# DongSky/few-shot-vit

Hardware: AMD Instinct MI355X
Metric: episodes_per_sec_5way_5shot_visformer_s (higher is better)
Workload: dtype bf16; 1 GPU; BASELINE configs[1]: Visformer-S (visformer_micro_80) miniImageNet-shaped 5-way 5-shot episodic eval, 15 query/class, 80x80 fp32 NCHW episodes resident in HBM, procedural weights + calibrated BN; images_per_episode=100, encoder_chunk_images=12800, distinct_episode_batches=16, parallelism=episode-parallel x1, one all-reduce of accuracy stats, ranks_seen=1, per_rank_eps=4602.6

## Files before the change

few-shot-vit_amd/csrc/conv3x3_halo.hip:

```cpp
#include <stdlib.h>

#include <type_traits>
#include <utility>

#include "conv_gemm.h"
#include "fsvit_common.h"

namespace FSVIT_NS {

__device__ __attribute__((aligned(256))) unsigned char g_zero_page_halo[256];
typedef __attribute__((address_space(3))) void* lptrh_t;

__device__ __forceinline__ void hdma1(const void* gsrc, unsigned lds_byte_addr) {
  unsigned keep;
  asm volatile(
      "s_mov_b32 %0, m0\n\t"
      "s_mov_b32 m0, %2\n\t"
      "s_nop 0\n\t"
      "global_load_lds_dwordx4 %1, off\n\t"
      "s_mov_b32 m0, %0"
      : "=&s"(keep)
      : "v"(gsrc), "s"(lds_byte_addr)
      : "memory");
}
__device__ __forceinline__ void hdma2s(unsigned off0, unsigned off1, const void* sbase, unsigned lds0, unsigned lds1) {
  unsigned keep;
  asm volatile(
      "s_mov_b32 %0, m0\n\t"
      "s_mov_b32 m0, %4\n\t"
      "s_nop 0\n\t"
      "global_load_lds_dwordx4 %1, %3\n\t"
      "s_mov_b32 m0, %5\n\t"
      "s_nop 0\n\t"
      "global_load_lds_dwordx4 %2, %3\n\t"
      "s_mov_b32 m0, %0"
      : "=&s"(keep)
      : "v"(off0), "v"(off1), "s"(sbase), "s"(lds0), "s"(lds1)
      : "memory");
}
__device__ __forceinline__ u32x4 hgload16(const void* p) {
  u32x4 v;
  asm volatile("global_load_dwordx4 %0, %1, off" : "=v"(v) : "v"(p) : "memory");
  return v;
}
#define HWAIT(vm) asm volatile("s_waitcnt vmcnt(" #vm ") lgkmcnt(0)" ::: "memory")
__device__ __forceinline__ void hbar() {
  asm volatile("s_barrier" ::: "memory");
  __builtin_amdgcn_sched_barrier(0);
}

template <int CTRL>
__device__ __forceinline__ float quad_xor(float v) {
  return __builtin_bit_cast(float, __builtin_amdgcn_update_dpp(0, __builtin_bit_cast(int, v), CTRL, 0xf, 0xf, true));
}

namespace halo {
constexpr int TR = 8, TW = 40;
constexpr int HR = TR + 2, HP = 44;
constexpr int PLANE = 7168;
constexpr int NPIECE = 7;
constexpr int HBUF = 8 * PLANE;
constexpr int NST = 3, STAGE = 16384;
constexpr int OFF_W = 2 * HBUF;
constexpr int LDS_BYTES = OFF_W + NST * STAGE;
static_assert(LDS_BYTES == 160 * 1024, "the two halo buffers and the weight ring fill the LDS exactly");
}

template <int... I, typename F>
__device__ __forceinline__ void static_for_impl(std::integer_sequence<int, I...>, F&& f) {
  (f(std::integral_constant<int, I>{}), ...);
}
template <int N, typename F>
__device__ __forceinline__ void static_for(F&& f) { static_for_impl(std::make_integer_sequence<int, N>{}, static_cast<F&&>(f)); }

template <int CIN, bool FUSE_TAIL, bool STATS = false>
__global__ __launch_bounds__(512, 2) void conv3x3_halo_kernel(const ConvGemmParams p, const int n_tiles) {
  using namespace halo;
  extern __shared__ __attribute__((aligned(16))) unsigned char smem[];
  constexpr int NH = CIN / 64;
  constexpr int NKM = 9 * NH, NKT = NKM + (FUSE_TAIL ? 1 : 0);
  constexpr int MT = 5, NT = 4;
  const int t = threadIdx.x, lane = t & 63;
  const int wave = __builtin_amdgcn_readfirstlane(t >> 6);
  const int wm = wave >> 1, wn = wave & 1;
  const int lrow = lane & 15, lq = lane >> 4;
  const unsigned lds0 = (unsigned)(size_t)(lptrh_t)smem;
  unsigned char* const wst0 = smem + OFF_W;

  const unsigned char* const Xb = reinterpret_cast<const unsigned char*>(p.x);
  const unsigned char* const Wb = reinterpret_cast<const unsigned char*>(p.w);
  bf16* __restrict__ Y = reinterpret_cast<bf16*>(p.y);
  const int tiles_per_img = p.H / TR;

  const int fr = ((lrow >> 3) & 1) * 2 + ((lrow >> 1) & 1), fc = ((lrow >> 2) & 1) * 2 + (lrow & 1);
  auto blk_r = [&](int i) { return (wm * MT + i) / (TW / 4); };
  auto blk_c = [&](int i) { return (wm * MT + i) % (TW / 4); };
  f32x4 st0[STATS ? NT : 1], st1[STATS ? NT : 1];
#pragma unroll
  for (int j = 0; j < (STATS ? NT : 1); ++j) st0[j] = st1[j] = f32x4{0.f, 0.f, 0.f, 0.f};
  unsigned xb[MT];
#pragma unroll
  for (int i = 0; i < MT; ++i) xb[i] = (unsigned)(((blk_r(i) * 4 + fr) * HP + blk_c(i) * 4 + fc) * 16 + lq * PLANE);
  const int srow = lane >> 3;
  const unsigned schunk = (unsigned)(((lane & 7) ^ srow) << 4);
  unsigned offB[2];
#pragma unroll
  for (int j = 0; j < 2; ++j) {
    const int R = (2 * wave + j) * 8 + srow;
    const int ch = (R & ~31) + 8 * ((R & 15) >> 2) + 4 * ((R >> 4) & 1) + (R & 3);
    offB[j] = (unsigned)ch * (unsigned)(p.Kw * 2) + schunk;
  }
  const unsigned b_rd = (unsigned)((wn * 64 + lrow) * 128);
  const unsigned sw0 = (unsigned)((lq ^ (lrow & 7)) << 4), sw1 = (unsigned)(((4 + lq) ^ (lrow & 7)) << 4);

  auto issue_w = [&](int wk, int stage) {
    const unsigned d = lds0 + OFF_W + stage * STAGE;
    hdma2s(offB[0], offB[1], Wb + (size_t)wk * 128, d + (2 * wave) * 1024, d + (2 * wave + 1) * 1024);
  };
  const int x_rs = p.x_planar ? (CIN / 8) * p.W * 16 : p.W * CIN * 2, x_ps = p.x_planar ? 16 : CIN * 2;
  auto issue_piece = [&](int j, int lane_o, const unsigned char* base, bool top, bool bot, int nb) {
    const int s = j * 64 + lane_o, hr = s / HP, hc = s - hr * HP;
    const bool ok = (base != nullptr) & (s < HR * HP) & (hc >= 1) & (hc <= TW) & !(top & (hr == 0)) & !(bot & (hr == HR - 1));
    const unsigned long a = (unsigned long)base + (unsigned long)(unsigned)(hr * x_rs + (hc - 1) * x_ps);
    const unsigned long z = (unsigned long)g_zero_page_halo;
    hdma1(reinterpret_cast<const void*>(ok ? a : z), lds0 + nb * HBUF + wave * PLANE + j * 1024);
  };
  auto halo_base = [&](int tile, int h) {
    const int bb = tile / tiles_per_img, rr = (tile - bb * tiles_per_img) * TR;
    return Xb + (long)(bb * p.H + rr - 1) * x_rs + (p.x_planar ? (h * 8 + wave) * p.W * 16 : h * 128 + wave * 16);
  };

  f32x4 acc[MT][NT];
#pragma unroll
  for (int i = 0; i < MT; ++i)
#pragma unroll
    for (int j = 0; j < NT; ++j) acc[i][j] = f32x4{0.f, 0.f, 0.f, 0.f};

  int tix = blockIdx.x;
  if (tix >= n_tiles) return;
  const int my_tiles = (n_tiles - tix + (int)gridDim.x - 1) / (int)gridDim.x;
  int steps_left = my_tiles * NKT;

  auto wk_of = [&](int q) { return q >= NKM ? NKM : (NH == 2 ? (q >= 9 ? (q - 9) * 2 + 1 : q * 2) : q); };

  {
    const int r00 = (tix % tiles_per_img) * TR;
    const unsigned char* b0 = halo_base(tix, 0);
#pragma unroll
    for (int j = 0; j < NPIECE; ++j) issue_piece(j, lane, b0, r00 == 0, r00 + TR == p.H, 0);
  }
  issue_w(wk_of(0), 0);
  issue_w(wk_of(1 % NKT), 1);
  HWAIT(0);
  hbar();
  int st_cur = 0, st_pre = 2, q_pre = 2 % NKT;
  int buf = 0;
#define H_STAMP(acc_)

  auto advance = [&]() {
    st_cur = st_cur == NST - 1 ? 0 : st_cur + 1;
    st_pre = st_pre == NST - 1 ? 0 : st_pre + 1;
    q_pre = q_pre == NKT - 1 ? 0 : q_pre + 1;
    --steps_left;
  };

  while (true) {
    const int tnext = tix + (int)gridDim.x;
    const bool has_next = tnext < n_tiles;
    const int b = tix / tiles_per_img, r0 = (tix - b * tiles_per_img) * TR;
    u32x4 xf0[MT], wf0[NT];

#pragma unroll 1
    for (int h = 0; h < NH; ++h) {
      const int n_tix = h + 1 < NH ? tix : (has_next ? tnext : -1), n_h = h + 1 < NH ? h + 1 : 0;
      const unsigned char* nbase = n_tix >= 0 ? halo_base(n_tix, n_h) : nullptr;
      const int n_r0 = n_tix >= 0 ? (n_tix % tiles_per_img) * TR : 0;
      const bool n_top = n_r0 == 0, n_bot = n_r0 + TR == p.H;
      int lane_o = lane;
      asm volatile("" : "+v"(lane_o));
      u32x4 xf1[MT], wf1[NT];
      {
        const unsigned char* wb = wst0 + st_cur * STAGE + b_rd;
#pragma unroll
        for (int j = 0; j < NT; ++j) wf0[j] = *reinterpret_cast<const u32x4*>(wb + j * 2048 + sw0);
#pragma unroll
        for (int i = 0; i < MT; ++i) xf0[i] = *reinterpret_cast<const u32x4*>(smem + xb[i]);
      }
      H_STAMP(ckP);
      static_for<9>([&](auto tapc) {
        constexpr int TAP = decltype(tapc)::value;
        constexpr int TOFF = ((TAP / 3) * HP + TAP % 3) * 16;
        constexpr int TOFF_N = (((TAP + 1) / 3) * HP + (TAP + 1) % 3) * 16;
        const bool pre_w = steps_left > 2;
        if (pre_w) issue_w(wk_of(q_pre), st_pre);
        __builtin_amdgcn_sched_barrier(0);
        {
          const unsigned char* wb = wst0 + st_cur * STAGE + b_rd;
#pragma unroll
          for (int j = 0; j < NT; ++j) wf1[j] = *reinterpret_cast<const u32x4*>(wb + j * 2048 + sw1);
#pragma unroll
          for (int i = 0; i < MT; ++i) xf1[i] = *reinterpret_cast<const u32x4*>(smem + xb[i] + 4 * PLANE + TOFF);
        }
#pragma unroll
        for (int i = 0; i < MT; ++i)
#pragma unroll
          for (int j = 0; j < NT; ++j) acc[i][j] = mma_chunk<bf16>(wf0[j], xf0[i], acc[i][j]);
#pragma unroll
        for (int k = 0; k < MT + NT; ++k) {
          __builtin_amdgcn_sched_group_barrier(0x008, 1, 0);
          __builtin_amdgcn_sched_group_barrier(0x100, 1, 0);
        }
        __builtin_amdgcn_sched_group_barrier(0x008, MT * NT - (MT + NT), 0);
        __builtin_amdgcn_sched_barrier(0);
        H_STAMP(ckA);
        if (TAP >= 1 && TAP <= NPIECE) { if (pre_w) HWAIT(3); else HWAIT(1); }
        else { if (pre_w) HWAIT(2); else HWAIT(0); }
        H_STAMP(ckV);
        hbar();
        H_STAMP(ckW);
        if constexpr (TAP < NPIECE) issue_piece(TAP, lane_o, nbase, n_top, n_bot, buf ^ 1);
        const int st_next = st_cur == NST - 1 ? 0 : st_cur + 1;
        if constexpr (TAP < 8) {
          const unsigned char* wb = wst0 + st_next * STAGE + b_rd;
#pragma unroll
          for (int j = 0; j < NT; ++j) wf0[j] = *reinterpret_cast<const u32x4*>(wb + j * 2048 + sw0);
#pragma unroll
          for (int i = 0; i < MT; ++i) xf0[i] = *reinterpret_cast<const u32x4*>(smem + xb[i] + TOFF_N);
        } else if (FUSE_TAIL) {
          if (h == NH - 1) {
            const bf16* X2 = reinterpret_cast<const bf16*>(p.x2);
#pragma unroll
            for (int i = 0; i < MT; ++i) {
              const int lr = lane_o & 15;
              const int fr_o = ((lr >> 3) & 1) * 2 + ((lr >> 1) & 1), fc_o = ((lr >> 2) & 1) * 2 + (lr & 1);
              const size_t pix = (size_t)(b * p.H + r0 + blk_r(i) * 4 + fr_o) * p.W + blk_c(i) * 4 + fc_o;
              xf0[i] = hgload16(X2 + pix * p.x2_cstride + lq * 8);
            }
          }
        }
#pragma unroll
        for (int i = 0; i < MT; ++i)
#pragma unroll
          for (int j = 0; j < NT; ++j) acc[i][j] = mma_chunk<bf16>(wf1[j], xf1[i], acc[i][j]);
        if constexpr (TAP < NPIECE) {
#pragma unroll
          for (int k = 0; k < 8; ++k) {
            __builtin_amdgcn_sched_group_barrier(0x008, 1, 0);
            __builtin_amdgcn_sched_group_barrier(0x002, 3, 0);
          }
#pragma unroll
          for (int k = 0; k < MT + NT; ++k) {
            __builtin_amdgcn_sched_group_barrier(0x008, 1, 0);
            __builtin_amdgcn_sched_group_barrier(0x100, 1, 0);
          }
          __builtin_amdgcn_sched_group_barrier(0x008, MT * NT - 8 - (MT + NT), 0);
        } else if constexpr (TAP < 8) {
#pragma unroll
          for (int k = 0; k < MT + NT; ++k) {
            __builtin_amdgcn_sched_group_barrier(0x008, 1, 0);
            __builtin_amdgcn_sched_group_barrier(0x100, 1, 0);
          }
          __builtin_amdgcn_sched_group_barrier(0x008, MT * NT - (MT + NT), 0);
        }
        __builtin_amdgcn_sched_barrier(0);
        H_STAMP(ckB);
        advance();
      });
      buf ^= 1;
#pragma unroll
      for (int i = 0; i < MT; ++i) xb[i] = buf ? xb[i] + (unsigned)HBUF : xb[i] - (unsigned)HBUF;
    }

    if constexpr (FUSE_TAIL) {
      asm volatile("s_waitcnt vmcnt(0)" : "+v"(xf0[0]), "+v"(xf0[1]), "+v"(xf0[2]), "+v"(xf0[3]), "+v"(xf0[4]) :: "memory");
      const bool pre_w = steps_left > 2;
      if (pre_w) issue_w(wk_of(q_pre), st_pre);
      {
        const unsigned char* wb = wst0 + st_cur * STAGE + b_rd;
#pragma unroll
        for (int j = 0; j < NT; ++j) wf0[j] = *reinterpret_cast<const u32x4*>(wb + j * 2048 + sw0);
      }
      __builtin_amdgcn_sched_barrier(0);
#pragma unroll
      for (int i = 0; i < MT; ++i)
#pragma unroll
        for (int j = 0; j < NT; ++j) acc[i][j] = mma_chunk<bf16>(wf0[j], xf0[i], acc[i][j]);
      __builtin_amdgcn_sched_barrier(0);
      asm volatile("s_waitcnt lgkmcnt(0)" ::: "memory");
      hbar();
      advance();
      H_STAMP(ckT);
    }

    {
      int lane_e = lane;
      asm volatile("" : "+v"(lane_e));
      const int lrow_e = lane_e & 15, lq_e = lane_e >> 4;
      const int fr_e = ((lrow_e >> 3) & 1) * 2 + ((lrow_e >> 1) & 1), fc_e = ((lrow_e >> 2) & 1) * 2 + (lrow_e & 1);
      f32x4 bv[NT];
#pragma unroll
      for (int j = 0; j < NT; ++j)
        bv[j] = p.bias ? *reinterpret_cast<const f32x4*>(p.bias + wn * 64 + (j >> 1) * 32 + lq_e * 8 + (j & 1) * 4) : f32x4{0.f, 0.f, 0.f, 0.f};
      if constexpr (STATS) {
#pragma unroll
        for (int i = 0; i < MT; ++i)
#pragma unroll
          for (int j = 0; j < NT; ++j) {
            const f32x4 v = acc[i][j] + bv[j];
            st0[j] += v;
            st1[j] += v * v;
          }
      }
      auto finish = [&](auto actf) {
#pragma unroll
        for (int i = 0; i < MT; ++i) {
          size_t orow;
          const float* posrow = nullptr;
          const int prow_i = blk_r(i) * 4 + fr_e, pcol_i = blk_c(i) * 4 + fc_e;
          if (FUSE_TAIL) {
            const int ph = p.H >> 1, pw = p.W >> 1;
            const int py = (r0 + prow_i) >> 1, px = pcol_i >> 1;
            orow = (size_t)(b * ph + py) * pw + px;
            posrow = p.pos + (size_t)(py * pw + px) * p.y_cstride;
          } else {
            orow = (size_t)(b * p.H + r0 + prow_i) * p.W + pcol_i;
          }
#pragma unroll
          for (int jp = 0; jp < NT / 2; ++jp) {
            const int n = wn * 64 + jp * 32 + lq_e * 8;
            f32x4 v[2];
#pragma unroll
            for (int u = 0; u < 2; ++u) {
              v[u] = acc[i][2 * jp + u] + bv[2 * jp + u];
              acc[i][2 * jp + u] = f32x4{0.f, 0.f, 0.f, 0.f};
#pragma unroll
              for (int e = 0; e < 4; ++e) v[u][e] = actf(v[u][e]);
              if (FUSE_TAIL) {
#pragma unroll
                for (int e = 0; e < 4; ++e) {
                  v[u][e] = fmaxf(v[u][e], quad_xor<0xB1>(v[u][e]));
                  v[u][e] = fmaxf(v[u][e], quad_xor<0x4E>(v[u][e]));
                }
                v[u] += *reinterpret_cast<const f32x4*>(posrow + n + 4 * u);
              }
            }
            if (!FUSE_TAIL || (lrow_e & 3) == 0) {
              const bf16x8 o = {(bf16)v[0][0], (bf16)v[0][1], (bf16)v[0][2], (bf16)v[0][3], (bf16)v[1][0], (bf16)v[1][1], (bf16)v[1][2], (bf16)v[1][3]};
              if (!FUSE_TAIL && p.y_planar) *reinterpret_cast<bf16x8*>(Y + (((size_t)(b * p.H + r0 + prow_i) * (p.y_cstride >> 3) + (n >> 3)) * p.W + pcol_i) * 8) = o;
              else *reinterpret_cast<bf16x8*>(Y + orow * p.y_cstride + n) = o;
            }
          }
        }
      };
      auto finish_pooled = [&](auto actf) {
        const int u_e = lrow_e & 3;
        const int nq = wn * 64 + (u_e >> 1) * 32 + lq_e * 8 + (u_e & 1) * 4;
        const f32x4 bq = p.bias ? *reinterpret_cast<const f32x4*>(p.bias + nq) : f32x4{0.f, 0.f, 0.f, 0.f};
        const int ph = p.H >> 1, pw = p.W >> 1;
#pragma unroll
        for (int i = 0; i < MT; ++i) {
          const int py = (r0 + blk_r(i) * 4 + fr_e) >> 1, px = (blk_c(i) * 4 + fc_e) >> 1;
          const f32x4 pq = *reinterpret_cast<const f32x4*>(p.pos + (size_t)(py * pw + px) * p.y_cstride + nq);
          f32x4 m[NT];
#pragma unroll
          for (int j = 0; j < NT; ++j) {
            m[j] = acc[i][j];
            acc[i][j] = f32x4{0.f, 0.f, 0.f, 0.f};
#pragma unroll
            for (int e = 0; e < 4; ++e) {
              m[j][e] = fmaxf(m[j][e], quad_xor<0xB1>(m[j][e]));
              m[j][e] = fmaxf(m[j][e], quad_xor<0x4E>(m[j][e]));
            }
          }
          f32x4 v = u_e == 0 ? m[0] : (u_e == 1 ? m[1] : (u_e == 2 ? m[2] : m[3]));
          v += bq;
#pragma unroll
          for (int e = 0; e < 4; ++e) v[e] = actf(v[e]);
          v += pq;
          store4<bf16>(Y + ((size_t)(b * ph + py) * pw + px) * p.y_cstride + nq, v);
        }
      };
      if (FUSE_TAIL && p.act == ACT_LRELU) finish_pooled([](float x) { return fmaxf(x, 0.1f * x); });
      else if (FUSE_TAIL && p.act == ACT_NONE) finish_pooled([](float x) { return x; });
      else if (p.act == ACT_GELU) finish([](float x) { return gelu_sig(x); });
      else if (p.act == ACT_LRELU) finish([](float x) { return fmaxf(x, 0.1f * x); });
      else finish([](float x) { return x; });
    }
    H_STAMP(ckE);
    if (!has_next) break;
    tix = tnext;
  }
  asm volatile("s_waitcnt vmcnt(0)" ::: "memory");
  if constexpr (STATS) {
    __syncthreads();
    float* red = reinterpret_cast<float*>(smem);
#pragma unroll
    for (int j = 0; j < NT; ++j)
#pragma unroll
      for (int e = 0; e < 4; ++e) {
        float a = st0[j][e], q = st1[j][e];
#pragma unroll
        for (int o = 1; o < 16; o <<= 1) { a += __shfl_xor(a, o); q += __shfl_xor(q, o); }
        if (lrow == 0) {
          const int cl = (j >> 1) * 32 + lq * 8 + (j & 1) * 4 + e;
          red[(wave * 2 + 0) * 64 + cl] = a;
          red[(wave * 2 + 1) * 64 + cl] = q;
        }
      }
    __syncthreads();
    if (t < 256) {
      const int which = t >> 7, c = t & 127, h = c >> 6, cl = c & 63;
      float a = 0.f;
#pragma unroll
      for (int m = 0; m < 4; ++m) a += red[((m * 2 + h) * 2 + which) * 64 + cl];
      p.stats[((size_t)blockIdx.x * 2 + which) * p.y_cstride + c] = a;
    }
  }
}

bool conv3x3_halo_eligible(const ConvGemmParams& p, int dtype) {
  constexpr bool off = false;
  if (off || dtype != 1) return false;
  if (p.KH != 3 || p.KW != 3 || p.stride != 1 || p.pad != 1 || p.groups != 1) return false;
  if (p.N != 128 || p.y_cstride != 128 || p.W != halo::TW || (p.H % halo::TR) || p.OH != p.H || p.OW != p.W) return false;
  if (p.res || p.y2 || p.act == ACT_MUL || p.y_rpi || p.out_f32 || p.w_rstride || p.w_gstride) return false;
  if (p.Cin != p.x_cstride || p.K != 9 * p.Cin) return false;
  if (p.stats && (p.pool2 || p.act != ACT_NONE)) return false;
  if (p.y_planar && (p.pool2 || p.stats)) return false;
  if (p.pool2) return p.Cin == 128 && p.x2 && p.K2 == 32 && p.x2_cstride >= 32 && p.pos && p.Kw == p.K + 64;
  return (p.Cin == 64 || p.Cin == 128) && !p.x2 && !p.pos && p.Kw == p.K;
}

static inline int halo_grid(const ConvGemmParams& p) { const int n_tiles = p.B * (p.H / halo::TR); return n_tiles < 256 ? n_tiles : 256; }
int conv3x3_halo_stats_rows(const ConvGemmParams& p, int dtype) {
  ConvGemmParams q = p;
  float dummy;
  q.stats = &dummy;
  return conv3x3_halo_eligible(q, dtype) ? halo_grid(p) : 0;
}

template <int CIN, bool FUSE_TAIL, bool STATS = false>
static int launch_halo_t(const ConvGemmParams& p, hipStream_t stream) {
  const int n_tiles = p.B * (p.H / halo::TR);
  auto kern = conv3x3_halo_kernel<CIN, FUSE_TAIL, STATS>;
  hipError_t e = hipFuncSetAttribute((const void*)kern, hipFuncAttributeMaxDynamicSharedMemorySize, halo::LDS_BYTES);
  if (e != hipSuccess) return (int)e;
  const int grid = n_tiles < 256 ? n_tiles : 256;
  hipLaunchKernelGGL(kern, dim3(grid), dim3(512), halo::LDS_BYTES, stream, p, n_tiles);
  return (int)hipGetLastError();
}

int launch_conv3x3_halo(const ConvGemmParams& p, hipStream_t stream) {
  if (p.pool2) return launch_halo_t<128, true>(p, stream);
  if (p.stats) return p.Cin == 64 ? launch_halo_t<64, false, true>(p, stream) : launch_halo_t<128, false, true>(p, stream);
  return p.Cin == 64 ? launch_halo_t<64, false>(p, stream) : launch_halo_t<128, false>(p, stream);
}

}
```

Baseline: 4599 episodes/s.

## Add weight-stationary 3x3 conv kernel for Cin=64 layers

Adds a new 3x3 convolution kernel that keeps all filter fragments resident in accumulation registers per wave and streams double-buffered input row groups into LDS via direct global-to-LDS loads. Each workgroup processes a persistent range of 4-row groups, prefetching the next group while computing MFMAs on the current one. The halo dispatcher routes eligible Cin=64 non-stats, non-pool layers to it, avoiding repeated weight reloads. The cost is heavy register pressure and one wave per SIMD occupancy. The non-f16 path also drops the Cin=64 fallback, which now returns an error.

```diff
diff --git a/few-shot-vit_amd/csrc/conv3x3_halo.hip b/few-shot-vit_amd/csrc/conv3x3_halo.hip
--- a/few-shot-vit_amd/csrc/conv3x3_halo.hip
+++ b/few-shot-vit_amd/csrc/conv3x3_halo.hip
@@ -450,10 +450,23 @@
   return (int)hipGetLastError();
 }
 
+#ifndef FSVIT_HALF_F16
+bool conv3x3_ws_eligible(const ConvGemmParams& p);
+int launch_conv3x3_ws(const ConvGemmParams& p, hipStream_t stream);
+
+int launch_conv3x3_halo(const ConvGemmParams& p, hipStream_t stream) {
+  if (conv3x3_ws_eligible(p)) return launch_conv3x3_ws(p, stream);
+  if (p.pool2) return launch_halo_t<128, true>(p, stream);
+  if (p.stats) return p.Cin == 64 ? launch_halo_t<64, false, true>(p, stream) : launch_halo_t<128, false, true>(p, stream);
+  if (p.Cin == 128) return launch_halo_t<128, false>(p, stream);
+  return (int)hipErrorInvalidValue;
+}
+#else
 int launch_conv3x3_halo(const ConvGemmParams& p, hipStream_t stream) {
   if (p.pool2) return launch_halo_t<128, true>(p, stream);
   if (p.stats) return p.Cin == 64 ? launch_halo_t<64, false, true>(p, stream) : launch_halo_t<128, false, true>(p, stream);
   return p.Cin == 64 ? launch_halo_t<64, false>(p, stream) : launch_halo_t<128, false>(p, stream);
 }
-
-}
+#endif
+
+}
diff --git a/few-shot-vit_amd/csrc/conv3x3_ws.hip b/few-shot-vit_amd/csrc/conv3x3_ws.hip
--- /dev/null
+++ b/few-shot-vit_amd/csrc/conv3x3_ws.hip
@@ -0,0 +1,311 @@
+#include <stdlib.h>
+
+#include <type_traits>
+#include <utility>
+
+#include "conv_gemm.h"
+#include "fsvit_common.h"
+
+namespace FSVIT_NS {
+
+#ifndef FSVIT_HALF_F16
+
+__device__ __attribute__((aligned(256))) unsigned char g_zero_page_ws[256];
+
+namespace ws3 {
+constexpr int GR = 4, W = 40;
+constexpr int PP = 42;
+constexpr int NX2 = 10;
+template <int CIN> struct Geo {
+  static constexpr int NPL = CIN / 8;
+  static constexpr int RS = NPL * PP + 8;
+  static constexpr int WSLOT = 6 * RS;
+  static constexpr int NPW = (WSLOT + 63) / 64;
+  static_assert(RS % 16 == 8, "row pitch must be 8 mod 16 slots");
+};
+}
+
+typedef float f32x16w __attribute__((ext_vector_type(16)));
+typedef __attribute__((address_space(3))) void* lptrw_t;
+
+template <int... I, typename F>
+__device__ __forceinline__ void ws_for_impl(std::integer_sequence<int, I...>, F&& f) {
+  (f(std::integral_constant<int, I>{}), ...);
+}
+template <int N, typename F>
+__device__ __forceinline__ void ws_for(F&& f) { ws_for_impl(std::make_integer_sequence<int, N>{}, static_cast<F&&>(f)); }
+
+__device__ __forceinline__ void ws_mfma(const u32x4& w, const u32x4& x, f32x16w& c) {
+  asm volatile(FSVIT_MFMA_32x32x16 " %0, %1, %2, %0" : "+v"(c) : "a"(w), "v"(x));
+}
+__device__ __forceinline__ void ws_mfma_z(const u32x4& w, const u32x4& x, f32x16w& c) {
+  asm volatile(FSVIT_MFMA_32x32x16 " %0, %1, %2, 0" : "=&v"(c) : "a"(w), "v"(x));
+}
+__device__ __forceinline__ void ws_mfma_vw(const u32x4& w, const u32x4& x, f32x16w& c) {
+  asm volatile(FSVIT_MFMA_32x32x16 " %0, %1, %2, %0" : "+v"(c) : "v"(w), "v"(x));
+}
+__device__ __forceinline__ void ws_dma(const void* gsrc, unsigned lds_byte_addr) {
+  unsigned keep;
+  asm volatile(
+      "s_mov_b32 %0, m0\n\t"
+      "s_mov_b32 m0, %2\n\t"
+      "s_nop 0\n\t"
+      "global_load_lds_dwordx4 %1, off\n\t"
+      "s_mov_b32 m0, %0"
+      : "=&s"(keep)
+      : "v"(gsrc), "s"(lds_byte_addr)
+      : "memory");
+}
+__device__ __forceinline__ void ws_st16(void* p, u32x4 v) {
+  asm volatile("s_nop 0\n\tglobal_store_dwordx4 %0, %1, off\n\ts_nop 0" :: "v"(p), "v"(v) : "memory");
+}
+__device__ __forceinline__ void ws_st8(void* p, u32x2 v) {
+  asm volatile("s_nop 0\n\tglobal_store_dwordx2 %0, %1, off" :: "v"(p), "v"(v) : "memory");
+}
+
+template <int CTRL>
+__device__ __forceinline__ float ws_quad(float v) {
+  return __builtin_bit_cast(float, __builtin_amdgcn_update_dpp(0, __builtin_bit_cast(int, v), CTRL, 0xf, 0xf, true));
+}
+__device__ __forceinline__ unsigned ws_pk2(float a, float b) {
+  typedef __attribute__((ext_vector_type(2))) bf16 bf16x2_t;
+  const bf16x2_t v = {(bf16)a, (bf16)b};
+  return __builtin_bit_cast(unsigned, v);
+}
+
+template <int CIN, int EPI, int ACT>
+__global__ __launch_bounds__(256, 1) void conv3x3_ws_kernel(const ConvGemmParams p, const int n_groups, const int per_wg) {
+  using namespace ws3;
+  using G = Geo<CIN>;
+  constexpr bool TAIL = EPI == 1;
+  constexpr int NKC = CIN / 16;
+  constexpr int NS = 9 * NKC + (TAIL ? 2 : 0);
+  constexpr int NPT = G::NPW + (TAIL ? NX2 : 0);
+  constexpr int NPWV = (NPT + 3) / 4;
+  constexpr int BUFB = 4 * NPWV * 1024;
+  constexpr int OFF_X2 = G::NPW * 1024;
+  constexpr int NSTORE = TAIL ? 5 : 10;
+  constexpr int NWA = NS < 64 ? NS : 64;
+  static_assert(2 * BUFB <= 160 * 1024, "two buffers must fit the LDS");
+  extern __shared__ __attribute__((aligned(16))) unsigned char smem[];
+
+  const int t = threadIdx.x, lane = t & 63, p5 = lane & 31, kh = lane >> 5;
+  const int wave = __builtin_amdgcn_readfirstlane(t >> 6);
+  const int g0 = blockIdx.x * per_wg;
+  const int g1 = g0 + per_wg < n_groups ? g0 + per_wg : n_groups;
+  if (g0 >= g1) return;
+  const unsigned lds0 = (unsigned)(size_t)(lptrw_t)smem;
+  const int gpi = p.H / GR;
+
+  const int cR = 16 * ((p5 >> 2) & 1) + 4 * (p5 >> 3) + (p5 & 3);
+  const bf16* const wrow = reinterpret_cast<const bf16*>(p.w) + (size_t)(32 * wave + cR) * p.Kw + 8 * kh;
+  u32x4 wf[NWA];
+#pragma unroll
+  for (int f = 0; f < NWA; ++f) wf[f] = *reinterpret_cast<const u32x4*>(wrow + (f / NKC) * CIN + 16 * (f % NKC));
+#pragma unroll
+  for (int f = 0; f < NWA; ++f) asm volatile("" : "+a"(wf[f]));
+
+  auto pix_r = [&](int b) { const int k = 8 * b + (p5 >> 2); return 2 * (k / 20) + ((p5 >> 1) & 1); };
+  auto pix_c = [&](int b) { const int k = 8 * b + (p5 >> 2); return 2 * (k % 20) + (p5 & 1); };
+  unsigned xb[5], xt[5];
+#pragma unroll
+  for (int b = 0; b < 5; ++b) {
+    xb[b] = (unsigned)((pix_r(b) * G::RS + kh * PP + pix_c(b)) * 16);
+    xt[b] = (unsigned)(OFF_X2 + (kh * 160 + pix_r(b) * W + pix_c(b)) * 16);
+  }
+
+  const unsigned char* const Xb = reinterpret_cast<const unsigned char*>(p.x);
+  const long rowb = (long)p.W * CIN * 2;
+  const int plane_b = p.x_planar ? p.W * 16 : 16, col_b = p.x_planar ? 16 : CIN * 2;
+  unsigned pk[NPWV];
+#pragma unroll
+  for (int i = 0; i < NPWV; ++i) {
+    const int j = wave + 4 * i;
+    unsigned v = 0u;
+    if (j < G::NPW) {
+      const int s = 64 * j + lane, row = s / G::RS, w = s - row * G::RS, pl = w / PP, cs = w - pl * PP;
+      const bool ok = (s < G::WSLOT) & (pl < G::NPL) & (cs >= 1) & (cs <= W);
+      v = ok ? (unsigned)(row * rowb + pl * plane_b + (cs - 1) * col_b) | ((unsigned)row << 16) | (1u << 19) : 0u;
+    } else if (TAIL) {
+      const int s = 64 * (j - G::NPW) + lane, c4 = s / 160, px = s - c4 * 160;
+      v = c4 < 4 ? (unsigned)(px * p.x2_cstride * 2 + c4 * 16) | (1u << 16) | (1u << 19) : 0u;
+    }
+    pk[i] = v;
+  }
+  struct Src { unsigned long bw, bt; bool top, bot, valid; };
+  auto src_of = [&](int gg, bool valid) {
+    const int bi = gg / gpi, r0 = (gg - bi * gpi) * GR;
+    Src r;
+    r.bw = (unsigned long)(Xb + (long)(bi * p.H + r0 - 1) * rowb);
+    r.bt = TAIL ? (unsigned long)p.x2 + (unsigned long)((long)(bi * p.H + r0) * p.W * p.x2_cstride * 2) : 0ul;
+    r.top = r0 == 0;
+    r.bot = r0 + GR == p.H;
+    r.valid = valid;
+    return r;
+  };
+  auto issue_piece = [&](int i, const Src& sr, int nb) {
+    const int j = wave + 4 * i;
+    const unsigned long base = (TAIL && j >= G::NPW) ? sr.bt : sr.bw;
+    const unsigned v = pk[i], row = (v >> 16) & 7u;
+    const bool ok = sr.valid & ((v >> 19) & 1u) & !(sr.top & (row == 0u)) & !(sr.bot & (row == 5u));
+    const unsigned long a = ok ? base + (v & 0xffffu) : (unsigned long)g_zero_page_ws;
+    ws_dma(reinterpret_cast<const void*>(a), lds0 + nb * BUFB + j * 1024);
+  };
+
+  {
+    const Src s0 = src_of(g0, true);
+#pragma unroll 1
+    for (int i = 0; i < NPWV; ++i) issue_piece(i, s0, 0);
+  }
+  asm volatile("s_waitcnt vmcnt(0)\n\ts_barrier" ::: "memory");
+  __builtin_amdgcn_sched_barrier(0);
+
+  f32x16w acc[5];
+  int buf = 0;
+  bf16* __restrict__ Y = reinterpret_cast<bf16*>(p.y);
+#pragma unroll 1
+  for (int gg = g0; gg < g1; ++gg) {
+    const bool has_next = gg + 1 < g1;
+    const int bi = gg / gpi, r0 = (gg - bi * gpi) * GR;
+    const unsigned cb = (unsigned)(buf * BUFB);
+    const Src sn = src_of(has_next ? gg + 1 : gg, has_next);
+    f32x4 bq[4];
+    auto load_epi = [&]() {
+      if constexpr (TAIL) {
+        const int nq = 32 * wave + 16 * kh + 4 * (lane & 3);
+        bq[0] = p.bias ? *reinterpret_cast<const f32x4*>(p.bias + nq) : f32x4{0.f, 0.f, 0.f, 0.f};
+      } else {
+#pragma unroll
+        for (int e = 0; e < 4; ++e)
+          bq[e] = p.bias ? *reinterpret_cast<const f32x4*>(p.bias + 32 * wave + 16 * kh + 4 * e) : f32x4{0.f, 0.f, 0.f, 0.f};
+      }
+    };
+
+    u32x4 xf[2][5];
+    constexpr int NWV = NS - NWA;
+    u32x4 wv[NWV > 0 ? NWV : 1];
+    auto load_wv = [&]() {
+      const bf16* wr = wrow;
+      asm volatile("" : "+v"(wr));
+#pragma unroll
+      for (int f = 0; f < NWV; ++f) wv[f] = *reinterpret_cast<const u32x4*>(wr + ((NWA + f) / NKC) * CIN + 16 * ((NWA + f) % NKC));
+    };
+    auto read_step = [&](auto sc, int slot) {
+      constexpr int S = decltype(sc)::value;
+      if constexpr (S < 9 * NKC) {
+        constexpr int tp = S / NKC, kc = S % NKC;
+        constexpr unsigned OFF = (unsigned)(((tp / 3) * G::RS + 2 * kc * PP + tp % 3) * 16);
+#pragma unroll
+        for (int b = 0; b < 5; ++b) xf[slot][b] = *reinterpret_cast<const u32x4*>(smem + cb + xb[b] + OFF);
+      } else {
+        constexpr unsigned OFF = (unsigned)(2 * (S - 9 * NKC) * 160 * 16);
+#pragma unroll
+        for (int b = 0; b < 5; ++b) xf[slot][b] = *reinterpret_cast<const u32x4*>(smem + cb + xt[b] + OFF);
+      }
+    };
+    read_step(std::integral_constant<int, 0>{}, 0);
+    ws_for<NS>([&](auto sc) {
+      constexpr int S = decltype(sc)::value;
+      if constexpr (S < NPWV) issue_piece(S, sn, buf ^ 1);
+      if constexpr (S == NS - 6) load_epi();
+      if constexpr (NWV > 0 && S == (NWA > 24 ? NWA - 24 : 0)) load_wv();
+      if constexpr (S + 1 < NS) read_step(std::integral_constant<int, S + 1>{}, (S + 1) & 1);
+      u32x4 w;
+      if constexpr (S < NWA) w = wf[S];
+      else w = wv[S - NWA];
+#pragma unroll
+      for (int b = 0; b < 5; ++b) {
+        if constexpr (S == 0) ws_mfma_z(w, xf[0][b], acc[b]);
+        else if constexpr (S < NWA) ws_mfma(w, xf[S & 1][b], acc[b]);
+        else ws_mfma_vw(w, xf[S & 1][b], acc[b]);
+      }
+    });
+    asm volatile("s_nop 7\n\ts_nop 7" : "+v"(acc[0]), "+v"(acc[1]), "+v"(acc[2]), "+v"(acc[3]), "+v"(acc[4]));
+
+    auto act = [](float x) {
+      if constexpr (ACT == ACT_LRELU) return fmaxf(x, 0.1f * x);
+      else if constexpr (ACT == ACT_GELU) return gelu_sig(x);
+      else return x;
+    };
+    if constexpr (TAIL) {
+      const int q = lane & 3;
+      const int ph = p.H >> 1, pw = p.W >> 1;
+      const int nq = 32 * wave + 16 * kh + 4 * q;
+#pragma unroll
+      for (int b = 0; b < 5; ++b) {
+        const int k = 8 * b + (p5 >> 2);
+        const int py = (r0 >> 1) + k / 20, px = k % 20;
+        const f32x4 pq = *reinterpret_cast<const f32x4*>(p.pos + (size_t)(py * pw + px) * p.y_cstride + nq);
+        f32x16w m = acc[b];
+#pragma unroll
+        for (int e = 0; e < 16; ++e) {
+          m[e] = fmaxf(m[e], ws_quad<0xB1>(m[e]));
+          m[e] = fmaxf(m[e], ws_quad<0x4E>(m[e]));
+        }
+        f32x4 v;
+#pragma unroll
+        for (int e = 0; e < 4; ++e) v[e] = q == 0 ? m[e] : (q == 1 ? m[4 + e] : (q == 2 ? m[8 + e] : m[12 + e]));
+        v += bq[0];
+#pragma unroll
+        for (int e = 0; e < 4; ++e) v[e] = act(v[e]);
+        v += pq;
+        ws_st8(Y + ((size_t)(bi * ph + py) * pw + px) * p.y_cstride + nq, u32x2{ws_pk2(v[0], v[1]), ws_pk2(v[2], v[3])});
+      }
+    } else {
+#pragma unroll
+      for (int b = 0; b < 5; ++b) {
+        const int row = r0 + pix_r(b), col = pix_c(b);
+        unsigned o[8];
+#pragma unroll
+        for (int e = 0; e < 8; ++e) o[e] = ws_pk2(act(acc[b][2 * e] + bq[e >> 1][(2 * e) & 3]), act(acc[b][2 * e + 1] + bq[e >> 1][(2 * e + 1) & 3]));
+        const int n = 32 * wave + 16 * kh;
+        bf16* y0;
+        size_t step;
+        if (p.y_planar) {
+          y0 = Y + (((size_t)(bi * p.H + row) * (p.y_cstride >> 3) + (n >> 3)) * p.W + col) * 8;
+          step = (size_t)p.W * 8;
+        } else {
+          y0 = Y + ((size_t)(bi * p.H + row) * p.W + col) * p.y_cstride + n;
+          step = 8;
+        }
+        ws_st16(y0, u32x4{o[0], o[1], o[2], o[3]});
+        ws_st16(y0 + step, u32x4{o[4], o[5], o[6], o[7]});
+      }
+    }
+    asm volatile("s_waitcnt vmcnt(%0) lgkmcnt(0)\n\ts_barrier" :: "n"(NSTORE) : "memory");
+    __builtin_amdgcn_sched_barrier(0);
+    buf ^= 1;
+  }
+  asm volatile("s_waitcnt vmcnt(0)" ::: "memory");
+}
+
+bool conv3x3_ws_eligible(const ConvGemmParams& p) {
+  if (p.stats || p.pool2 || p.Cin != 64 || (p.H % ws3::GR)) return false;
+  return p.act == ACT_NONE || p.act == ACT_LRELU || p.act == ACT_GELU;
+}
+
+template <int CIN, int EPI, int ACT>
+static int launch_ws_t(const ConvGemmParams& p, hipStream_t stream) {
+  using namespace ws3;
+  constexpr int NPT = Geo<CIN>::NPW + (EPI == 1 ? NX2 : 0);
+  constexpr int LDS = 2 * 4 * ((NPT + 3) / 4) * 1024;
+  const int n_groups = p.B * (p.H / GR);
+  int grid = n_groups < 256 ? n_groups : 256;
+  const int per = (n_groups + grid - 1) / grid;
+  grid = (n_groups + per - 1) / per;
+  auto kern = conv3x3_ws_kernel<CIN, EPI, ACT>;
+  hipError_t e = hipFuncSetAttribute((const void*)kern, hipFuncAttributeMaxDynamicSharedMemorySize, LDS);
+  if (e != hipSuccess) return (int)e;
+  hipLaunchKernelGGL(kern, dim3(grid), dim3(256), LDS, stream, p, n_groups, per);
+  return (int)hipGetLastError();
+}
+
+int launch_conv3x3_ws(const ConvGemmParams& p, hipStream_t stream) {
+  if (p.act == ACT_LRELU) return launch_ws_t<64, 0, ACT_LRELU>(p, stream);
+  if (p.act == ACT_GELU) return launch_ws_t<64, 0, ACT_GELU>(p, stream);
+  return launch_ws_t<64, 0, ACT_NONE>(p, stream);
+}
+
+#endif
+
+}
```

Result: no change. 4596 episodes/s (median of 6 runs) (-0.1%).
